# alexxx-db/dbx-distributed-pytorch-examples

Measured on AMD Instinct MI355X. Metric: images/sec (whole node) ResNet-50 ImageNet-1K at 1/2/4/8 MI355X; top-1 acc, higher is better.
Workload: dtype bf16; 1 GPU; model=resnet50 ImageNet-1K 224x224 1000 classes large-batch (global 8192 at 8 GPUs), global_batch=1024, per_gpu_batch=1024, parallelism=dp1, world_size_seen=1, backend=none, impl=native, optimizer=SGD momentum 0.9 nesterov=False wd 5e-5, memory_format=nhwc, graphs=True, ddp=none, kernels=dbx HIP (conv implicit-GEMM MFMA + fused BN/ReLU/pool/CE/SGD)

## Files before the change

### dbx_distributed_pytorch_examples_amd/csrc/abi.h

```cpp
#pragma once
typedef __bf16 bf16;
namespace dbx {
struct BnFin {
  unsigned* cnt;
  const double* stats;
  const float* gamma;
  const float* beta;
  float* running_mean;
  float* running_var;
  float* scale;
  float* shift;
  float* mean;
  float* invstd;
  float* coeff;
  float* dgamma;
  float* dbeta;
  int C, nshard, mode, accumulate;
  float count, eps, momentum, pad_;
};
struct IGemmArgs {
  const bf16* x;
  const bf16* w;
  bf16* y;
  const float* in_scale;
// ... 9 lines not shown
  const bf16* ybn;
  const bf16* ybn2;
  const float* bsc;
  const float* bsh;
  const float* mean1;
  const float* inv1;
  const float* mean2;
  const float* inv2;
  double* bstats1;
  double* bstats2;
  bf16* a_out;
  const bf16* res;
  const float* res_scale;
  const float* res_shift;
  bf16* tail_out;
  unsigned char* tail_bits;
  unsigned long long mag_ohw, mag_ow;
  const BnFin* fin1;
  const BnFin* fin2;
  int fin_base, fin_final;
  const BnFin* fin_in;
  float* skws;
  unsigned* skcnt;
  int ksplit, kper;
};
struct WgradArgs {
  const bf16* dy;
  const bf16* x;
  float* ws;
  const float* in_scale;
  const float* in_shift;
  int N, IH, IW, IC, OH, OW, OC, R, S, stride, pad;
  int M, KTOT, nsplit, m_per_split, relu_in;
  unsigned long long mag_ow, mag_ohw;
  float* dw;
  unsigned* cnt;
  float scale;
  int accumulate;
};
struct DwFusedArgs {
  const bf16* g;
  const bf16* y3;
  const float* coeff;
  const bf16* wt;
  const bf16* y2;
  const float* bsc;
  const float* bsh;
  const float* mean2;
  const float* inv2;
  bf16* da;
  double* bstats;
  float* ws;
  int M, K, C, nshard;
};
struct StemBwdArgs {
  const bf16* dpool;
  const unsigned char* arg;
  const bf16* y;
  const float* sc;
  const float* sh;
  const float* coeff;
  const bf16* x4;
  float* ws;
  int N, H, W, C, P, Q, PK, pstride, ppad;
  int IH, IW, R, S, stride, pad;
  int M, nsplit, m_per_split;
  unsigned long long mag_hw, mag_w;
};
struct GemmArgs {
  const bf16* A;
  const bf16* B;
  void* C;
  const float* bias_f;
  const bf16* bias_h;
  int M, N, K, lda, ldb, ldc;
  float alpha;
  int accumulate;
  unsigned long long seed;
  unsigned offset, thresh;
  float inv_keep;
  const unsigned* offset_dev;
  float* ws;
  int splitk;
};

}
```

### dbx_distributed_pytorch_examples_amd/csrc/bindings.cpp

```cpp
#include <hip/hip_runtime.h>
#include <pybind11/pybind11.h>
#include <pybind11/stl.h>
#include <stdint.h>

#include <stdexcept>
#include <string>

namespace py = pybind11;
#include "abi.h"

extern "C" {
int dbx_conv_igemm(int mode, int bm, int bn, const dbx::IGemmArgs* a, int pro, int stats, int accum, int epi,
                   hipStream_t st, int dma);
int dbx_conv_wgrad(int mode, int bm, int bn, const dbx::WgradArgs* a, int pro, hipStream_t st, unsigned lds_pad,
                   int dma);
int dbx_wgrad_reduce_multi_plan(const float* const*, float* const*, const long long*, const int*, const float*,
                                const int*, int, void*, int*, int*);
int dbx_wgrad_reduce_multi_run(const void*, int, int, int, hipStream_t);
int dbx_wgrad_reduce_job_bytes();
int dbx_wgrad_reduce(const float* ws, float* dw, long long n, int nsplit, float scale, int accumulate, hipStream_t st);
int dbx_wgrad_reduce_gather(const float* ws, float* dw, int OC, int R, int S, int IC, int nsplit, float scale,
                            int accumulate, hipStream_t st);
int dbx_wgrad_patch3(const dbx::WgradArgs* a, long long ws_cap, hipStream_t st, int max_wg);
int dbx_conv_dwfused(const dbx::DwFusedArgs* a, long long ws_cap, hipStream_t st, int max_cus);
// ... 105 lines not shown
    if (fin2 && !bstats2) throw std::invalid_argument("conv_igemm: second BN finalize without its statistics");
    {
      const unsigned long long two40 = 1ull << 40, ohw = (unsigned long long)OH * OW;
      if (ohw > 0 && (unsigned long long)N * ohw * ohw < two40) {
        a.mag_ohw = (two40 + ohw - 1) / ohw;
        a.mag_ow = (two40 + OW - 1) / OW;
      }
    }
    check(dbx_conv_igemm(mode, bm, bn, &a, in_scale != 0, stats != 0, accum, epi, S(st), dma), "conv_igemm");
  });
  m.def("wgrad_reduce_multi_plan", [](std::vector<uintptr_t> ws, std::vector<uintptr_t> dw, std::vector<long long> n,
                                       std::vector<int> nsplit, std::vector<float> scale, std::vector<int> acc,
                                       uintptr_t table) {
    const size_t nj = ws.size();
    if (dw.size() != nj || n.size() != nj || nsplit.size() != nj || scale.size() != nj || acc.size() != nj)
      throw std::invalid_argument("wgrad_reduce_multi_plan: job lists of different lengths");
    std::vector<const float*> w(nj);
    std::vector<float*> d(nj);
    for (size_t q = 0; q < nj; ++q) { w[q] = P<const float*>(ws[q]); d[q] = P<float*>(dw[q]); }
    int ga = 0, gb = 0;
    check(dbx_wgrad_reduce_multi_plan(w.data(), d.data(), n.data(), nsplit.data(), scale.data(), acc.data(), (int)nj,
                                      P<void*>(table), &ga, &gb),
          "wgrad_reduce_multi_plan");
    return std::make_pair(ga, gb);
  });
  m.def("wgrad_reduce_multi_run", [](uintptr_t table_dev, int nj, int ga, int gb, uintptr_t st) {
    check(dbx_wgrad_reduce_multi_run(P<const void*>(table_dev), nj, ga, gb, S(st)), "wgrad_reduce_multi_run");
  });
  m.def("wgrad_reduce_job_bytes", []() { return dbx_wgrad_reduce_job_bytes(); });
  m.def("conv_wgrad", [](int mode, int bm, int bn, uintptr_t dy, uintptr_t x, uintptr_t ws, uintptr_t in_scale,
                         uintptr_t in_shift, int relu_in, int N, int IH, int IW, int IC, int OH, int OW, int OC, int R,
                         int S_, int stride, int pad, int KTOT, int nsplit, int m_per_split, uintptr_t st,
                         unsigned lds_pad, int dma, uintptr_t dw, uintptr_t cnt, float scale, int accumulate) {
    const unsigned long long two40 = 1ull << 40;
    const unsigned long long ohw = (unsigned long long)OH * OW;
    if ((unsigned long long)N * ohw * ohw >= two40) throw std::runtime_error("conv_wgrad: batch too large for mdiv");
    dbx::WgradArgs a{P<const bf16*>(dy), P<const bf16*>(x), P<float*>(ws), P<const float*>(in_scale),
                     P<const float*>(in_shift), N, IH, IW, IC, OH, OW, OC, R, S_, stride, pad, N * OH * OW, KTOT,
                     nsplit, m_per_split, relu_in, (two40 + OW - 1) / OW, (two40 + ohw - 1) / ohw,
                     P<float*>(dw), P<unsigned*>(cnt), scale, accumulate};
    if (dw && nsplit > 1 && !cnt) throw std::invalid_argument("conv_wgrad: fused split-K reduction needs tile counters");
    check(dbx_conv_wgrad(mode, bm, bn, &a, in_scale != 0, S(st), lds_pad, dma), "conv_wgrad");
  });
  m.def("wgrad_patch3", [](uintptr_t dy, uintptr_t x, uintptr_t ws, long long ws_cap, int N, int IH, int IW, int IC,
                           int OH, int OW, int OC, int R, int S_, int stride, int pad, uintptr_t st, int max_wg) {
    dbx::WgradArgs a{P<const bf16*>(dy), P<const bf16*>(x), P<float*>(ws), nullptr, nullptr, N, IH, IW, IC, OH, OW,
                     OC, R, S_, stride, pad, N * OH * OW, R * S_ * IC, 0, 0, 0, 0ull, 0ull};
    const int n = dbx_wgrad_patch3(&a, ws_cap, S(st), max_wg);
    if (n <= 0) check(n ? n : -1, "wgrad_patch3");
    return n;
  });
  m.def("conv_dwfused", [](uintptr_t g, uintptr_t y3, uintptr_t coeff, uintptr_t wt, uintptr_t y2, uintptr_t bsc,
                           uintptr_t bsh, uintptr_t mean2, uintptr_t inv2, uintptr_t da, uintptr_t bstats, uintptr_t ws,
                           long long ws_cap, int M, int K, int C, int nshard, uintptr_t st, int max_cus) {
    dbx::DwFusedArgs a{P<const bf16*>(g), P<const bf16*>(y3), P<const float*>(coeff), P<const bf16*>(wt),
                       P<const bf16*>(y2), P<const float*>(bsc), P<const float*>(bsh), P<const float*>(mean2),
                       P<const float*>(inv2), P<bf16*>(da), P<double*>(bstats), P<float*>(ws), M, K, C,
                       nshard > 0 ? nshard : 1};
    const int n = dbx_conv_dwfused(&a, ws_cap, S(st), max_cus);
    if (n <= 0) check(n ? n : -1, "conv_dwfused");
    return n;
  });
  m.def("stem_bwd", [](uintptr_t dpool, uintptr_t arg, uintptr_t y, uintptr_t sc, uintptr_t sh, uintptr_t coeff,
                       uintptr_t x4, uintptr_t ws, long long ws_cap, int N, int H, int W, int C, int Pp, int Qq, int PK,
                       int pstride, int ppad, int IH, int IW, int R, int S_, int stride, int pad, int fused,
                       uintptr_t st) {
    const unsigned long long two40 = 1ull << 40, hw = (unsigned long long)H * W;
    if ((unsigned long long)N * hw * hw >= two40) throw std::runtime_error("stem_bwd: batch too large for mdiv");
    dbx::StemBwdArgs a{P<const bf16*>(dpool), P<const unsigned char*>(arg), P<const bf16*>(y), P<const float*>(sc),
                       P<const float*>(sh), P<const float*>(coeff), P<const bf16*>(x4), P<float*>(ws), N, H, W, C, Pp, Qq,
                       PK, pstride, ppad, IH, IW, R, S_, stride, pad, N * H * W, 0, 0, (two40 + hw - 1) / hw,
                       (two40 + W - 1) / W};
    const int n = dbx_stem_bwd(&a, ws_cap, fused, S(st));
    if (n <= 0) check(n ? n : -1, "stem_bwd");
    return n;
  });
  m.def("wgrad_reduce_gather", [](uintptr_t ws, uintptr_t dw, int OC, int R, int S_, int IC, int nsplit, float scale,
                                  int acc, uintptr_t st) {
    check(dbx_wgrad_reduce_gather(P<const float*>(ws), P<float*>(dw), OC, R, S_, IC, nsplit, scale, acc, S(st)),
          "wgrad_reduce_gather");
  });
  m.def("wgrad_reduce", [](uintptr_t ws, uintptr_t dw, long long n, int nsplit, float scale, int acc, uintptr_t st) {
    check(dbx_wgrad_reduce(P<const float*>(ws), P<float*>(dw), n, nsplit, scale, acc, S(st)), "wgrad_reduce");
  });
  m.def("bn_finalize", [](uintptr_t stats, int nshard, int C, float count, uintptr_t gamma, uintptr_t beta, float eps,
                          float momentum, uintptr_t rm, uintptr_t rv, uintptr_t scale, uintptr_t shift, uintptr_t smean,
                          uintptr_t sinv, uintptr_t st) {
    check(dbx_bn_finalize(P<const double*>(stats), nshard, C, count, P<const float*>(gamma), P<const float*>(beta), eps,
                          momentum, P<float*>(rm), P<float*>(rv), P<float*>(scale), P<float*>(shift), P<float*>(smean),
                          P<float*>(sinv), S(st)),
          "bn_finalize");
  });
  m.def("bn_eval_coeff", [](int C, uintptr_t gamma, uintptr_t beta, float eps, uintptr_t rm, uintptr_t rv,
                            uintptr_t scale, uintptr_t shift, uintptr_t st) {
    check(dbx_bn_eval_coeff(C, P<const float*>(gamma), P<const float*>(beta), eps, P<const float*>(rm),
                            P<const float*>(rv), P<float*>(scale), P<float*>(shift), S(st)),
          "bn_eval_coeff");
  });
  m.def("bn_eval_coeff_multi", [](uintptr_t desc, int nbn, int max_c, uintptr_t st) {
    check(dbx_bn_eval_coeff_multi(P<const void*>(desc), nbn, max_c, S(st)), "bn_eval_coeff_multi");
  });
  m.def("ce_eval", [](uintptr_t logits, int is_bf16, uintptr_t labels, uintptr_t stats, int B, int C, int k,
                      uintptr_t nvalid, uintptr_t loss_out, uintptr_t rank_out, uintptr_t st) {
    check(dbx_ce_eval(P<const void*>(logits), is_bf16, P<const long long*>(labels), P<double*>(stats), B, C, k,
                      P<const int*>(nvalid), P<float*>(loss_out), P<int*>(rank_out), S(st)),
          "ce_eval");
  });
  m.def("channel_stats", [](uintptr_t y, long long M, int C, uintptr_t stats, int nshard, uintptr_t st) {
    check(dbx_channel_stats(P<const bf16*>(y), M, C, P<double*>(stats), nshard, S(st)), "channel_stats");
  });
  m.def("bn_apply", [](uintptr_t y, uintptr_t sc, uintptr_t sh, uintptr_t res, uintptr_t rsc, uintptr_t rsh,
// ... 201 lines not shown
```

### dbx_distributed_pytorch_examples_amd/csrc/conv_dwfused.hip

```cpp
#include "common.h"
#include "abi.h"

namespace dbx {

template <int C, int NKB, int BM, int NS, int NT, int WN, int OCC, bool Y2N>
__global__ __launch_bounds__(NT, OCC) void dwfused_kernel(const DwFusedArgs a) {
  constexpr int K = NKB * 64;
  constexpr int NW = NT / 64, WM = NW / WN;
  constexpr int WC = C / WN;
  constexpr int WCH = K / 8;
  constexpr int CPR = C / 8;
  constexpr int RPP = NT / CPR;
  constexpr int NY = BM / RPP;
  constexpr int LR = NT / 8;
  constexpr int NG = BM / LR;
  constexpr int TM = BM / (16 * WM), TN = WC / 16;
  constexpr int TNW = WC / 16;
  static_assert(NKB % NS == 0 && C % 64 == 0 && WM == 2 && BM % (16 * WM) == 0 && BM % LR == 0 && BM % RPP == 0,
                "tile shape");
  constexpr int LDS_W = C * K, LDS_A = 2 * BM * 64, LDS_P = BM * C;
  static_assert(BM * (C + 8) <= LDS_A + LDS_P, "epilogue staging must fit the dy3 + a2 images");
  __shared__ __attribute__((aligned(16))) bf16 lds[LDS_W + LDS_A + LDS_P];
  bf16* sW = lds;
  bf16* sA = lds + LDS_W;
  bf16* sP = sA + LDS_A;
  bf16* sC = sA;

  const int tid = threadIdx.x, lane = tid & 63, wid = tid >> 6, wm = wid / WN, wn = wid % WN;
  const int ntile = a.M / BM;
  const int lrow = tid >> 3, lch = tid & 7;
  const int erow = tid / CPR, ech = tid % CPR;

  for (int q = tid; q < C * WCH; q += NT) {
    const int row = q / WCH, ch = q - (q / WCH) * WCH;
    *reinterpret_cast<u32x4*>(sW + row * K + ((ch ^ (row & 15)) << 3)) =
        *reinterpret_cast<const u32x4*>(a.wt + (size_t)row * K + ch * 8);
  }
  int cbn = ech * 8;
  auto bn2_affine = [&](f32x4& s0, f32x4& s1, f32x4& h0, f32x4& h1) __attribute__((always_inline)) {
    asm volatile("" : "+v"(cbn));
    s0 = *reinterpret_cast<const f32x4*>(a.bsc + cbn);
    s1 = *reinterpret_cast<const f32x4*>(a.bsc + cbn + 4);
    h0 = *reinterpret_cast<const f32x4*>(a.bsh + cbn);
    h1 = *reinterpret_cast<const f32x4*>(a.bsh + cbn + 4);
  };
  f32x2 st_s[4], st_q[4];
#pragma unroll
  for (int h = 0; h < 4; ++h) st_s[h] = st_q[h] = f32x2{0.f, 0.f};
  f32x4 accw[NKB][2][TNW];
#pragma unroll
  for (int kb = 0; kb < NKB; ++kb)
#pragma unroll
    for (int i = 0; i < 2; ++i)
#pragma unroll
      for (int j = 0; j < TNW; ++j) accw[kb][i][j] = f32x4{0.f, 0.f, 0.f, 0.f};

  const rsrc_t gr = make_rsrc(a.g, 2ull * a.M * K);
  const rsrc_t yr = make_rsrc(a.y3, 2ull * a.M * K);
  const rsrc_t y2r = make_rsrc(a.y2, 2ull * a.M * C);
  u32x4 rg[NS][NG], ry[NS][NG], ry2[NY], ry2n[Y2N ? NY : 1];
  auto load_k = [&](int t, int kb, int set) __attribute__((always_inline)) {
#pragma unroll
    for (int i = 0; i < NG; ++i) {
      const unsigned off = t < ntile ? 2u * (unsigned)((t * BM + lrow + LR * i) * K + kb * 64 + lch * 8) : kOOB;
      rg[set][i] = buf_load16(gr, off);
      ry[set][i] = buf_load16(yr, off);
    }
  };
  auto y2_off = [&](int t, int i) __attribute__((always_inline)) {
    return t < ntile ? 2u * (unsigned)((t * BM + erow + RPP * i) * C + ech * 8) : kOOB;
  };
  auto fold_store = [&](int kb, int buf, int set) __attribute__((always_inline)) {
    const int c0 = kb * 64 + lch * 8;
    const f32x4 k1a = *reinterpret_cast<const f32x4*>(a.coeff + c0);
    const f32x4 k1b = *reinterpret_cast<const f32x4*>(a.coeff + c0 + 4);
    const f32x4 k2a = *reinterpret_cast<const f32x4*>(a.coeff + K + c0);
    const f32x4 k2b = *reinterpret_cast<const f32x4*>(a.coeff + K + c0 + 4);
    const f32x4 k3a = *reinterpret_cast<const f32x4*>(a.coeff + 2 * K + c0);
    const f32x4 k3b = *reinterpret_cast<const f32x4*>(a.coeff + 2 * K + c0 + 4);
#pragma unroll
    for (int i = 0; i < NG; ++i) {
      float f[8], y[8];
      unpack8(rg[set][i], f);
      unpack8(ry[set][i], y);
#pragma unroll
      for (int j = 0; j < 4; ++j) {
        f[j] = f[j] * k1a[j] + k3a[j] + y[j] * k2a[j];
        f[j + 4] = f[j + 4] * k1b[j] + k3b[j] + y[j + 4] * k2b[j];
      }
      const int row = lrow + LR * i;
      *reinterpret_cast<u32x4*>(sA + buf * BM * 64 + row * 64 + (tr_swz(row, lch, 8) << 3)) = pack8(f);
    }
  };
  auto a2_store = [&]() __attribute__((always_inline)) {
    f32x4 bsc0, bsc1, bsh0, bsh1;
    bn2_affine(bsc0, bsc1, bsh0, bsh1);
#pragma unroll
    for (int i = 0; i < NY; ++i) {
      float f[8];
      unpack8(ry2[i], f);
#pragma unroll
      for (int j = 0; j < 4; ++j) {
        f[j] = f[j] * bsc0[j] + bsh0[j];
        f[j + 4] = f[j + 4] * bsc1[j] + bsh1[j];
      }
      const int row = erow + RPP * i;
      *reinterpret_cast<u32x4*>(sP + row * C + (tr_swz(row, ech, CPR) << 3)) = relu_bf16x8(pack8(f));
    }
  };

  const int g4 = lane >> 4, q4 = (lane & 15) >> 2, p4 = lane & 3;
  f32x4 accd[TM][TN];
  auto mma = [&](int kb, int buf) __attribute__((always_inline)) {
    const bf16* cA = sA + buf * BM * 64;
#pragma unroll
    for (int ks = 0; ks < 2; ++ks) {
      const int ch = ks * 4 + g4;
      bf16x8 af[TM], bw[TN];
#pragma unroll
      for (int i = 0; i < TM; ++i) {
        const int row = wm * (BM / WM) + i * 16 + (lane & 15);
        af[i] = *reinterpret_cast<const bf16x8*>(cA + row * 64 + (tr_swz(row, ch, 8) << 3));
      }
#pragma unroll
      for (int j = 0; j < TN; ++j) {
        const int crow = wn * WC + j * 16 + (lane & 15);
        bw[j] = *reinterpret_cast<const bf16x8*>(sW + crow * K + (((kb * 8 + ch) ^ (crow & 15)) << 3));
      }
#pragma unroll
      for (int i = 0; i < TM; ++i)
#pragma unroll
        for (int j = 0; j < TN; ++j)
          accd[i][j] = __builtin_amdgcn_mfma_f32_16x16x32_bf16(bw[j], af[i], accd[i][j], 0, 0, 0);
    }
#pragma unroll
    for (int ks = 0; ks < BM / 32; ++ks) {
      const int row = ks * 32 + 8 * g4 + q4, row2 = row + 4;
      bf16x8 af[2], bp[TNW];
#pragma unroll
      for (int i = 0; i < 2; ++i) {
        const int col = wm * 32 + i * 16 + 4 * p4;
        const s16x4 lo = __builtin_amdgcn_ds_read_tr16_b64_v4i16(
            (DBX_LDS s16x4*)(cA + row * 64 + (tr_swz(row, col >> 3, 8) << 3) + (col & 7)));
        const s16x4 hi = __builtin_amdgcn_ds_read_tr16_b64_v4i16(
            (DBX_LDS s16x4*)(cA + row2 * 64 + (tr_swz(row2, col >> 3, 8) << 3) + (col & 7)));
        af[i] = __builtin_bit_cast(bf16x8, __builtin_shufflevector(lo, hi, 0, 1, 2, 3, 4, 5, 6, 7));
      }
#pragma unroll
      for (int j = 0; j < TNW; ++j) {
        const int col = wn * WC + j * 16 + 4 * p4;
        const s16x4 lo = __builtin_amdgcn_ds_read_tr16_b64_v4i16(
            (DBX_LDS s16x4*)(sP + row * C + (tr_swz(row, col >> 3, CPR) << 3) + (col & 7)));
        const s16x4 hi = __builtin_amdgcn_ds_read_tr16_b64_v4i16(
            (DBX_LDS s16x4*)(sP + row2 * C + (tr_swz(row2, col >> 3, CPR) << 3) + (col & 7)));
        bp[j] = __builtin_bit_cast(bf16x8, __builtin_shufflevector(lo, hi, 0, 1, 2, 3, 4, 5, 6, 7));
      }
#pragma unroll
      for (int i = 0; i < 2; ++i)
#pragma unroll
        for (int j = 0; j < TNW; ++j)
          accw[kb][i][j] = __builtin_amdgcn_mfma_f32_16x16x32_bf16(af[i], bp[j], accw[kb][i][j], 0, 0, 0);
    }
  };

  int t = blockIdx.x;
#pragma unroll
  for (int i = 0; i < NY; ++i) ry2[i] = buf_load16(y2r, y2_off(t, i));
#pragma unroll
  for (int s = 0; s < NS; ++s) load_k(t, s, s);
  __syncthreads();
  for (; t < ntile; t += gridDim.x) {
    const int tn = t + gridDim.x;
    if constexpr (Y2N) {
#pragma unroll
      for (int i = 0; i < NY; ++i) ry2n[i] = buf_load16(y2r, y2_off(tn, i));
    }
    a2_store();
    fold_store(0, 0, 0);
    __syncthreads();
#pragma unroll
    for (int i = 0; i < TM; ++i)
#pragma unroll
      for (int j = 0; j < TN; ++j) accd[i][j] = f32x4{0.f, 0.f, 0.f, 0.f};
#pragma unroll
    for (int kb = 0; kb < NKB; ++kb) {
      const int f = kb + NS;
      load_k(f < NKB ? t : tn, f < NKB ? f : f - NKB, kb % NS);
      mma(kb, kb & 1);
      if (kb + 1 < NKB) fold_store(kb + 1, (kb + 1) & 1, (kb + 1) % NS);
      __syncthreads();
    }
#pragma unroll
    for (int i = 0; i < TM; ++i)
#pragma unroll
      for (int j = 0; j < TN; ++j) {
        const int row = wm * (BM / WM) + i * 16 + (lane & 15);
        const int col = wn * WC + j * 16 + g4 * 4;
        *reinterpret_cast<uint2*>(sC + row * (C + 8) + col) =
            uint2{pack2(accd[i][j][0], accd[i][j][1]), pack2(accd[i][j][2], accd[i][j][3])};
      }
    __syncthreads();
    f32x4 bsc0, bsc1, bsh0, bsh1;
    bn2_affine(bsc0, bsc1, bsh0, bsh1);
#pragma unroll
    for (int i = 0; i < NY; ++i) {
      const int row = erow + RPP * i;
      float f[8], y[8];
      unpack8(*reinterpret_cast<const u32x4*>(sC + row * (C + 8) + ech * 8), f);
      unpack8(ry2[i], y);
#pragma unroll
      for (int j = 0; j < 4; ++j) {
        const float t0 = y[j] * bsc0[j] + bsh0[j], t1 = y[j + 4] * bsc1[j] + bsh1[j];
        f[j] = t0 > 0.f ? f[j] : 0.f;
        f[j + 4] = t1 > 0.f ? f[j + 4] : 0.f;
      }
      const u32x4 v = pack8(f);
      *reinterpret_cast<u32x4*>(a.da + (size_t)(t * BM + row) * C + ech * 8) = v;
#pragma unroll
      for (int h = 0; h < 4; ++h) {
        const f32x2 gv = {__uint_as_float(v[h] << 16), __uint_as_float(v[h] & 0xFFFF0000u)};
        const f32x2 yv = {__uint_as_float(ry2[i][h] << 16), __uint_as_float(ry2[i][h] & 0xFFFF0000u)};
        st_s[h] += gv;
        st_q[h] = __builtin_elementwise_fma(gv, yv, st_q[h]);
      }
      if constexpr (Y2N) ry2[i] = ry2n[i];
      else ry2[i] = buf_load16(y2r, y2_off(tn, i));
    }
    __syncthreads();
  }

  float* out = a.ws + (size_t)blockIdx.x * K * C;
#pragma unroll
  for (int kb = 0; kb < NKB; ++kb)
#pragma unroll
    for (int i = 0; i < 2; ++i)
#pragma unroll
      for (int j = 0; j < TNW; ++j)
#pragma unroll
        for (int r = 0; r < 4; ++r) {
          const int k = kb * 64 + wm * 32 + i * 16 + g4 * 4 + r;
          out[(size_t)k * C + wn * WC + j * 16 + (lane & 15)] = accw[kb][i][j][r];
        }
  float s[8], q[8];
#pragma unroll
  for (int h = 0; h < 4; ++h) {
    s[2 * h] = st_s[h].x; s[2 * h + 1] = st_s[h].y;
    q[2 * h] = st_q[h].x; q[2 * h + 1] = st_q[h].y;
  }
#pragma unroll
  for (int j = 0; j < 8; ++j)
#pragma unroll
    for (int o = CPR; o < 64; o <<= 1) {
      s[j] += __shfl_xor(s[j], o, 64);
      q[j] += __shfl_xor(q[j], o, 64);
    }
  float* red = reinterpret_cast<float*>(sA);
  if (lane < CPR) {
#pragma unroll
    for (int j = 0; j < 8; ++j) {
      red[(wid * 2 + 0) * C + lane * 8 + j] = s[j];
      red[(wid * 2 + 1) * C + lane * 8 + j] = q[j];
    }
  }
  __syncthreads();
  for (int c = tid; c < C; c += NT) {
    float ss = 0.f, qq = 0.f;
#pragma unroll
    for (int w = 0; w < NW; ++w) { ss += red[(w * 2) * C + c]; qq += red[(w * 2 + 1) * C + c]; }
    qq = a.inv2[c] * (qq - a.mean2[c] * ss);
    double* st = a.bstats + (size_t)(blockIdx.x % a.nshard) * 2 * C;
    atomicAdd(st + c, (double)ss);
    atomicAdd(st + C + c, (double)qq);
  }
}

}

using namespace dbx;

template <int C, int NKB, int BM, int NS, int NT, int WN, int OCC, bool Y2N>
static int launch_dwfused(const DwFusedArgs& a, long long ws_cap, hipStream_t st, int max_cus) {
  if (a.M % BM != 0 || a.M <= 0) return -31;
  struct Occ { int per_cu, cus; };
  static const Occ occ = [] {
    int per_cu = 0, dev = 0, cus = 0;
    (void)hipOccupancyMaxActiveBlocksPerMultiprocessor(
        &per_cu, reinterpret_cast<const void*>(&dwfused_kernel<C, NKB, BM, NS, NT, WN, OCC, Y2N>), NT, 0);
    (void)hipGetDevice(&dev);
    (void)hipDeviceGetAttribute(&cus, hipDeviceAttributeMultiprocessorCount, dev);
    return Occ{per_cu, cus};
  }();
  const int cus = (max_cus > 0 && max_cus < occ.cus) ? (max_cus & ~7) : occ.cus;
  const int cap = (occ.per_cu > 0 && cus > 0) ? occ.per_cu * cus : 256;
  const int ntile = a.M / BM;
  const int grid = ntile < cap ? ntile : cap;
  if ((long long)(grid + (grid < 64 ? grid : 64)) * a.K * a.C > ws_cap) return -33;
  hipLaunchKernelGGL((dwfused_kernel<C, NKB, BM, NS, NT, WN, OCC, Y2N>), dim3(grid), dim3(NT), 0, st, a);
  const hipError_t e = hipGetLastError();
  return e == hipSuccess ? grid : -(int)e - 1000;
}

extern "C" int dbx_conv_dwfused(const DwFusedArgs* args, long long ws_cap, hipStream_t st, int max_cus) {
  const DwFusedArgs& a = *args;
  if (2ull * a.M * a.K >= (unsigned long long)kOOB) return -32;
#ifndef DBX_DWF64
#define DBX_DWF64 64, 2, 256, 2, 2, false
#endif
  if (a.C == 64 && a.K == 256) return launch_dwfused<64, 4, DBX_DWF64>(a, ws_cap, st, max_cus);
#ifndef DBX_DWF128
#define DBX_DWF128 64, 2, 256, 2, 1, false
#endif
  if (a.C == 128 && a.K == 512) return launch_dwfused<128, 8, DBX_DWF128>(a, ws_cap, st, max_cus);
  return -30;
}
```

### dbx_distributed_pytorch_examples_amd/ops/kernels.py

```python
from __future__ import annotations

import os
from typing import Optional, Tuple

import torch

from ..utils import debug as _debug
from . import reference as _ref
from ._ext import C, stream_ptr, use_native
from ..engine_config import EngineConfig

_E = EngineConfig.current

FWD, DGRAD, STEM, FWD_PATCH, DGRAD_PATCH = 0, 1, 2, 3, 4
_NO_EPI = (0, 1, 0, 0, 0, 0, 0, 0, 0, 0, 0, 0, 0, 0)
MASK_NONE, MASK_OUT, MASK_Y = 0, 1, 2


_POST_LAUNCH = None


def set_post_launch(cb, owner=None) -> None:
    global _POST_LAUNCH
    if cb is None and owner is not None and _POST_LAUNCH is not None and _POST_LAUNCH != owner:
# ... 683 lines not shown
                              cus=num_cus() - cu_reserve if cu_reserve > 0 else None)
    if (nsplit + (min(64, nsplit) if nsplit > 8 else 0)) * OC * KTOT > ws.numel():
        raise ValueError("wgrad workspace too small")
    fuse = not stem and (nsplit == 1 or (cnt is not None and nsplit * bm * bn * 4 <= wgrad_fuse_max()))
    if fuse and nsplit > 1:
        _chk(cnt, torch.int32, "cnt")
        if cnt.numel() < (OC // bm) * (KTOT // bn):
            raise ValueError("conv_wgrad: tile counter slice too small")
    region = None
    if (defer is not None and not fuse and (defer.max_slab_bytes is None
                                           or 4 * nsplit * OC * KTOT <= defer.max_slab_bytes)):
        region = defer.alloc((nsplit + (min(64, nsplit) if nsplit > 8 else 0)) * OC * KTOT)
        if region is not None:
            ws = region
    C().conv_wgrad(STEM if stem else FWD, bm, bn, dy.data_ptr(), x.data_ptr(), ws.data_ptr(), _p(in_scale),
                   _p(in_shift), int(relu_in), N, IH, IW, IC, OH, OW, OC, R, S, stride, pad, KTOT, nsplit, ms,
                   stream_ptr(), int(lds_pad), int(dma), dw.data_ptr() if fuse else 0,
                   cnt.data_ptr() if fuse and cnt is not None else 0, float(scale), int(accumulate))
    if region is not None:
        defer.add(ws, dw, OC * KTOT, nsplit, scale, accumulate)
    elif not fuse:
        C().wgrad_reduce(ws.data_ptr(), dw.data_ptr(), OC * KTOT, nsplit, float(scale), int(accumulate), stream_ptr())
    return dw


def dwfused_supported(C: int, K: int, M: int) -> bool:
    return (C, K) in ((64, 256), (128, 512)) and M % 64 == 0 and 2 * M * K < 0xFFFFFF00


def num_cus() -> int:
    global _NUM_CUS
    if _NUM_CUS is None:
        try:
            _NUM_CUS = int(torch.cuda.get_device_properties(torch.cuda.current_device()).multi_processor_count) \
                if torch.cuda.is_available() else 256
        except Exception:
            _NUM_CUS = 256
    return _NUM_CUS


_NUM_CUS = None


def dwfused_grid(C: int, K: int) -> int:
    return (2 if (C, K) == (64, 256) else 1) * num_cus()


def dwfused_preferred(C: int, K: int, M: int) -> bool:
    grid = dwfused_grid(C, K)
    return dwfused_supported(C, K, M) and M >= _E().fuse_dw_min_tiles * grid * 64


@_dispatch
def conv_dwfused(g, y3, coeff, wt16, y2, scale2, shift2, mean2, invstd2, bstats2, da, dw, ws, cus: int = 0):
    N, H, W, Kc = g.shape
    Cc = y2.shape[-1]
    M = N * H * W
    _chk(g, torch.bfloat16, "g")
    _chk(y3, torch.bfloat16, "y3", g.numel())
    _chk(coeff, torch.float32, "coeff", 3 * Kc)
    _chk(wt16, torch.bfloat16, "wt16", Cc * Kc)
    _chk(y2, torch.bfloat16, "y2", M * Cc)
    _chk(da, torch.bfloat16, "da", M * Cc)
    _chk(dw, torch.float32, "dw", Kc * Cc)
    _chk(ws, torch.float32, "ws")
    nsh2 = _chk_stats(bstats2, "bstats2", Cc)
    for t, nm in ((scale2, "scale2"), (shift2, "shift2"), (mean2, "mean2"), (invstd2, "invstd2")):
        _chk(t, torch.float32, nm, Cc)
    if not dwfused_supported(Cc, Kc, M):
        raise ValueError(f"conv_dwfused: unsupported geometry C={Cc} K={Kc} M={M}")
    n = C().conv_dwfused(g.data_ptr(), y3.data_ptr(), coeff.data_ptr(), wt16.data_ptr(), y2.data_ptr(),
                         scale2.data_ptr(), shift2.data_ptr(), mean2.data_ptr(), invstd2.data_ptr(), da.data_ptr(),
                         bstats2.data_ptr(), ws.data_ptr(), ws.numel(), M, Kc, Cc, nsh2, stream_ptr(), int(cus))
    C().wgrad_reduce(ws.data_ptr(), dw.data_ptr(), Kc * Cc, n, 1.0, 0, stream_ptr())
    return da


@_dispatch
def bn_finalize(stats, count, gamma, beta, eps, momentum, running_mean, running_var, scale, shift,
                save_mean, save_invstd):
    Cc = scale.numel()
    C().bn_finalize(stats.data_ptr(), _nsh(stats, Cc), Cc, float(count), _p(gamma), _p(beta), float(eps), float(momentum),
                    _p(running_mean), _p(running_var), scale.data_ptr(), shift.data_ptr(), _p(save_mean),
                    _p(save_invstd), stream_ptr())


@_dispatch
def bn_eval_coeff(gamma, beta, eps, running_mean, running_var, scale, shift):
    C().bn_eval_coeff(scale.numel(), _p(gamma), _p(beta), float(eps), running_mean.data_ptr(),
                      running_var.data_ptr(), scale.data_ptr(), shift.data_ptr(), stream_ptr())


def pack_bn_eval_desc(entries, device) -> torch.Tensor:
    import numpy as np
    want = torch.device(device)
    rows = np.zeros(len(entries), dtype=_ref.bn_eval_desc_dtype())
    for i, (gamma, beta, eps, rm, rv, scale, shift) in enumerate(entries):
        n = scale.numel()
        for t, nm in ((gamma, "gamma"), (beta, "beta"), (rm, "running_mean"), (rv, "running_var"), (scale, "scale"),
                      (shift, "shift")):
            if t is None and nm in ("gamma", "beta"):
                continue
            if t.dtype != torch.float32:
                raise TypeError(f"pack_bn_eval_desc: entry {i} {nm}: expected torch.float32, got {t.dtype}")
            same_dev = t.device.type == want.type and (want.index is None or t.device.index == want.index)
            if not t.is_contiguous() or not same_dev:
                raise ValueError(f"pack_bn_eval_desc: entry {i} {nm}: must be contiguous and on {device}")
            if t.numel() != n:
                raise ValueError(f"pack_bn_eval_desc: entry {i} {nm}: {t.numel()} elements, scale has {n}")
        rows[i] = ([_p(gamma), _p(beta), rm.data_ptr(), rv.data_ptr(), scale.data_ptr(), shift.data_ptr()], n, eps)
    table = torch.from_numpy(rows.view(np.uint8).copy()).to(device)
    return table, len(entries), max((int(r["C"]) for r in rows), default=0)


@_dispatch
def bn_eval_coeff_multi(desc, nbn, max_c):
    if desc.dtype != torch.uint8:
        raise TypeError(f"desc: expected torch.uint8, got {desc.dtype}")
    if not desc.is_contiguous() or desc.numel() != _ref.BN_EVAL_DESC_BYTES * int(nbn):
        raise ValueError(f"desc: expected a contiguous [{nbn}, {_ref.BN_EVAL_DESC_BYTES}] byte table, got shape "
                         f"{tuple(desc.shape)}")
    C().bn_eval_coeff_multi(desc.data_ptr(), int(nbn), int(max_c), stream_ptr())


@_dispatch
def channel_stats(y, stats):
# ... 539 lines not shown
```

### dbx_distributed_pytorch_examples_amd/ops/reference.py

```python
from __future__ import annotations

import math

import torch
import torch.nn.functional as F

NSHARD = 32
MASK_NONE, MASK_OUT, MASK_Y = 0, 1, 2


def check_channels(C: int) -> None:
    if C < 8 or C % 8 or C // 8 > 256:
        raise ValueError(f"per-channel kernels need a channel count that is a multiple of 8, at most 2048; got {C}")


def _shards(stats, C: int):
    n = stats.numel() // (2 * C)
    if n < 1 or n > 32 or n * 2 * C != stats.numel():
        raise ValueError(f"statistics slab of {stats.numel()} elements is not [nshard <= 32, 2, {C}]")
    return stats.view(n, 2, C)


def _nchw(x):
    return x.permute(0, 3, 1, 2)
# ... 73 lines not shown
        else:
            t = y * e.scale + e.shift
            g = g * (t > 0)
            if getattr(e, "act_out", None) is not None:
                e.act_out.copy_(torch.relu(t).bfloat16())
        g = g.bfloat16().float()
        gf = g.reshape(-1, Cc)
        st = e.stats1.view(-1, 2, Cc)
        st[0, 0] += gf.sum(0)
        st[0, 1] += (gf * ((y - e.mean1) * e.inv1).reshape(-1, Cc)).sum(0)
        if e.ybn2 is not None:
            st2 = e.stats2.view(-1, 2, Cc)
            st2[0, 0] += gf.sum(0)
            st2[0, 1] += (gf * ((e.ybn2.float() - e.mean2) * e.inv2).reshape(-1, Cc)).sum(0)
        if hasattr(e, "run_fin"):
            e.run_fin()
    dx.copy_(g.bfloat16())
    return dx


def conv_stem_fwd(x4, w16s, out, *, R=7, S=7, stride=2, pad=3, stats=None, patch=None):
    OC = w16s.shape[0]
    w = w16s.float().view(OC, 8, 8, 4)[:, :R, :S, :].permute(0, 3, 1, 2)
    y = _nhwc(F.conv2d(_nchw(x4.float()), w, stride=stride, padding=pad)).bfloat16()
    out.copy_(y)
    if stats is not None:
        _add_stats(stats, out)
    return out


def conv_wgrad(dy, x, dw, ws, *, R, S, stride, pad, in_scale=None, in_shift=None, relu_in=True, scale=1.0,
               accumulate=False, stem=False, tile=None, lds_pad=0, dma=-1, cnt=None, out_krsc=None, rounds=None,
               defer=None, cu_reserve=0):
    N, OH, OW, OC = dy.shape
    IC = x.shape[-1]
    xf = _act_in(x, in_scale, in_shift, relu_in)
    g = torch.nn.grad.conv2d_weight(_nchw(xf), (OC, IC, R, S), _nchw(dy.float()), stride=stride, padding=pad)
    g = g.permute(0, 2, 3, 1) * scale
    if stem and out_krsc is not None:
        icr = out_krsc.numel() // (OC * R * S)
        out_krsc.copy_((g[..., :icr].reshape(-1) + (out_krsc if accumulate else 0)))
        return out_krsc
    if stem:
        full = torch.zeros(OC, 8, 8, 4, dtype=torch.float32, device=dy.device)
        full[:, :R, :S, :IC] = g
        g = full
    g = g.reshape(dw.shape)
    if accumulate:
        g = g + dw
    dw.copy_(g)
    return dw


def conv_dwfused(g, y3, coeff, wt16, y2, scale2, shift2, mean2, invstd2, bstats2, da, dw, ws, cus=0):
    from types import SimpleNamespace
    dy = torch.empty_like(g)
    bn_bwd_apply(g, y3, coeff, dy, mask_mode=MASK_NONE)
    act = torch.relu(y2.float() * scale2 + shift2).bfloat16()
    epi = SimpleNamespace(mode=MASK_Y, ybn=y2, mean1=mean2, inv1=invstd2, stats1=bstats2, mbits=None, scale=scale2,
                          shift=shift2, ybn2=None, mean2=None, inv2=None, stats2=None, act_out=None)
    conv_dgrad(dy, wt16, da, R=1, S=1, stride=1, pad=0, epilogue=epi)
    conv_wgrad(dy, act, dw, ws, R=1, S=1, stride=1, pad=0)
    return da


def bn_finalize(stats, count, gamma, beta, eps, momentum, running_mean, running_var, scale, shift, save_mean,
                save_invstd):
    C = scale.numel()
    st = _shards(stats, C).double().sum(0)
    mean = st[0] / count
    var = (st[1] / count - mean * mean).clamp_min(0)
    invstd = 1.0 / torch.sqrt(var + eps)
    g = gamma.double() if gamma is not None else torch.ones_like(mean)
    b = beta.double() if beta is not None else torch.zeros_like(mean)
    scale.copy_((g * invstd).float())
    shift.copy_((b - mean * g * invstd).float())
    if save_mean is not None:
        save_mean.copy_(mean.float())
    if save_invstd is not None:
        save_invstd.copy_(invstd.float())
    if running_mean is not None and momentum > 0:
        unb = var * count / (count - 1) if count > 1 else var
        running_mean.mul_(1 - momentum).add_(momentum * mean.float())
        running_var.mul_(1 - momentum).add_(momentum * unb.float())


def bn_eval_coeff(gamma, beta, eps, running_mean, running_var, scale, shift):
    inv = torch.rsqrt(running_var + eps)
    g = gamma if gamma is not None else torch.ones_like(inv)
    b = beta if beta is not None else torch.zeros_like(inv)
    scale.copy_(g * inv)
    shift.copy_(b - running_mean * g * inv)


BN_EVAL_DESC_BYTES = 56


def bn_eval_desc_dtype():
    import numpy as np
    return np.dtype([("ptr", np.int64, (6,)), ("C", np.int32), ("eps", np.float32)])


def bn_eval_coeff_multi(desc, nbn, max_c):
    import ctypes
    if desc.dtype != torch.uint8 or desc.numel() != BN_EVAL_DESC_BYTES * int(nbn):
        raise ValueError("bn_eval_coeff_multi: expected a uint8 [nbn, 56] table")

# ... 569 lines not shown
```

Measured before the change: 17050 images/s.

## Split C=128 dwfused kernel into two channel-half slices with persistent slab walk

For the C=128, K=512 fused dgrad/wgrad backward kernel, the default path now launches a C=64-sliced variant in which paired blocks each handle one channel half of the same M tiles, walking slabs persistently. BN coefficients and scale/shift are staged in LDS, and the transposed activation fragments are loaded once per tile. The goal is to cut per-block LDS and register footprint and raise parallelism. The cost is that g/y3 loads and the fold work are repeated across the two halves. The old kernel remains reachable with variant=1.

Result: no change. 17130 images/s, median of 6 (+0.5%).

```diff
diff --git a/dbx_distributed_pytorch_examples_amd/csrc/abi.h b/dbx_distributed_pytorch_examples_amd/csrc/abi.h
--- a/dbx_distributed_pytorch_examples_amd/csrc/abi.h
+++ b/dbx_distributed_pytorch_examples_amd/csrc/abi.h
@@ -85,6 +85,8 @@
   double* bstats;
   float* ws;
   int M, K, C, nshard;
+  int variant;
+  int nwalk;
 };
 struct StemBwdArgs {
   const bf16* dpool;
diff --git a/dbx_distributed_pytorch_examples_amd/csrc/bindings.cpp b/dbx_distributed_pytorch_examples_amd/csrc/bindings.cpp
--- a/dbx_distributed_pytorch_examples_amd/csrc/bindings.cpp
+++ b/dbx_distributed_pytorch_examples_amd/csrc/bindings.cpp
@@ -181,11 +181,11 @@
   });
   m.def("conv_dwfused", [](uintptr_t g, uintptr_t y3, uintptr_t coeff, uintptr_t wt, uintptr_t y2, uintptr_t bsc,
                            uintptr_t bsh, uintptr_t mean2, uintptr_t inv2, uintptr_t da, uintptr_t bstats, uintptr_t ws,
-                           long long ws_cap, int M, int K, int C, int nshard, uintptr_t st, int max_cus) {
+                           long long ws_cap, int M, int K, int C, int nshard, uintptr_t st, int max_cus, int variant) {
     dbx::DwFusedArgs a{P<const bf16*>(g), P<const bf16*>(y3), P<const float*>(coeff), P<const bf16*>(wt),
                        P<const bf16*>(y2), P<const float*>(bsc), P<const float*>(bsh), P<const float*>(mean2),
                        P<const float*>(inv2), P<bf16*>(da), P<double*>(bstats), P<float*>(ws), M, K, C,
-                       nshard > 0 ? nshard : 1};
+                       nshard > 0 ? nshard : 1, variant};
     const int n = dbx_conv_dwfused(&a, ws_cap, S(st), max_cus);
     if (n <= 0) check(n ? n : -1, "conv_dwfused");
     return n;
diff --git a/dbx_distributed_pytorch_examples_amd/csrc/conv_dwfused.hip b/dbx_distributed_pytorch_examples_amd/csrc/conv_dwfused.hip
--- a/dbx_distributed_pytorch_examples_amd/csrc/conv_dwfused.hip
+++ b/dbx_distributed_pytorch_examples_amd/csrc/conv_dwfused.hip
@@ -3,14 +3,17 @@
 
 namespace dbx {
 
-template <int C, int NKB, int BM, int NS, int NT, int WN, int OCC, bool Y2N>
+template <int C, int NKB, int BM, int NS, int NT, int WN, int OCC, bool Y2N, int CT = C>
 __global__ __launch_bounds__(NT, OCC) void dwfused_kernel(const DwFusedArgs a) {
   constexpr int K = NKB * 64;
+  static_assert(CT == C || CT == 2 * C, "slicing");
+  constexpr bool SL = CT != C;
   constexpr int NW = NT / 64, WM = NW / WN;
   constexpr int WC = C / WN;
   constexpr int WCH = K / 8;
   constexpr int CPR = C / 8;
-  constexpr int RPP = NT / CPR;
+  constexpr int ET = SL ? 128 : NT;
+  constexpr int RPP = ET / CPR;
   constexpr int NY = BM / RPP;
   constexpr int LR = NT / 8;
   constexpr int NG = BM / LR;
@@ -20,44 +23,53 @@
                 "tile shape");
   constexpr int LDS_W = C * K, LDS_A = 2 * BM * 64, LDS_P = BM * C;
   static_assert(BM * (C + 8) <= LDS_A + LDS_P, "epilogue staging must fit the dy3 + a2 images");
-  __shared__ __attribute__((aligned(16))) bf16 lds[LDS_W + LDS_A + LDS_P];
+  constexpr int LDS_X = SL ? 2 * (3 * K + 2 * C) : 0;
+  __shared__ __attribute__((aligned(16))) bf16 lds[LDS_W + LDS_A + LDS_P + LDS_X];
   bf16* sW = lds;
   bf16* sA = lds + LDS_W;
   bf16* sP = sA + LDS_A;
   bf16* sC = sA;
+  float* sX = reinterpret_cast<float*>(sP + LDS_P);
 
   const int tid = threadIdx.x, lane = tid & 63, wid = tid >> 6, wm = wid / WN, wn = wid % WN;
   const int ntile = a.M / BM;
   const int lrow = tid >> 3, lch = tid & 7;
   const int erow = tid / CPR, ech = tid % CPR;
+  const bool ep = !SL || tid < ET;
+  const int half = SL ? (blockIdx.x >> 3) & 1 : 0;
+  int slab = SL ? ((blockIdx.x >> 4) << 3) + (blockIdx.x & 7) : blockIdx.x;
+  const int tstep = SL ? a.nwalk : gridDim.x;
+  const int coff = half * C;
+  if (SL && slab >= a.nwalk) return;
 
   for (int q = tid; q < C * WCH; q += NT) {
     const int row = q / WCH, ch = q - (q / WCH) * WCH;
     *reinterpret_cast<u32x4*>(sW + row * K + ((ch ^ (row & 15)) << 3)) =
-        *reinterpret_cast<const u32x4*>(a.wt + (size_t)row * K + ch * 8);
-  }
-  int cbn = ech * 8;
+        *reinterpret_cast<const u32x4*>(a.wt + (size_t)(coff + row) * K + ch * 8);
+  }
+  if constexpr (SL) {
+    for (int q = tid; q < 3 * K; q += NT) sX[q] = a.coeff[q];
+    for (int q = tid; q < C; q += NT) {
+      sX[3 * K + q] = a.bsc[coff + q];
+      sX[3 * K + C + q] = a.bsh[coff + q];
+    }
+  }
+  int cbn = SL ? 3 * K + ech * 8 : ech * 8;
+  const float* pbsc = SL ? sX : a.bsc;
+  const float* pbsh = SL ? sX + C : a.bsh;
   auto bn2_affine = [&](f32x4& s0, f32x4& s1, f32x4& h0, f32x4& h1) __attribute__((always_inline)) {
     asm volatile("" : "+v"(cbn));
-    s0 = *reinterpret_cast<const f32x4*>(a.bsc + cbn);
-    s1 = *reinterpret_cast<const f32x4*>(a.bsc + cbn + 4);
-    h0 = *reinterpret_cast<const f32x4*>(a.bsh + cbn);
-    h1 = *reinterpret_cast<const f32x4*>(a.bsh + cbn + 4);
+    s0 = *reinterpret_cast<const f32x4*>(pbsc + cbn);
+    s1 = *reinterpret_cast<const f32x4*>(pbsc + cbn + 4);
+    h0 = *reinterpret_cast<const f32x4*>(pbsh + cbn);
+    h1 = *reinterpret_cast<const f32x4*>(pbsh + cbn + 4);
   };
   f32x2 st_s[4], st_q[4];
-#pragma unroll
-  for (int h = 0; h < 4; ++h) st_s[h] = st_q[h] = f32x2{0.f, 0.f};
   f32x4 accw[NKB][2][TNW];
-#pragma unroll
-  for (int kb = 0; kb < NKB; ++kb)
-#pragma unroll
-    for (int i = 0; i < 2; ++i)
-#pragma unroll
-      for (int j = 0; j < TNW; ++j) accw[kb][i][j] = f32x4{0.f, 0.f, 0.f, 0.f};
 
   const rsrc_t gr = make_rsrc(a.g, 2ull * a.M * K);
   const rsrc_t yr = make_rsrc(a.y3, 2ull * a.M * K);
-  const rsrc_t y2r = make_rsrc(a.y2, 2ull * a.M * C);
+  const rsrc_t y2r = make_rsrc(a.y2, 2ull * a.M * CT);
   u32x4 rg[NS][NG], ry[NS][NG], ry2[NY], ry2n[Y2N ? NY : 1];
   auto load_k = [&](int t, int kb, int set) __attribute__((always_inline)) {
 #pragma unroll
@@ -68,16 +80,18 @@
     }
   };
   auto y2_off = [&](int t, int i) __attribute__((always_inline)) {
-    return t < ntile ? 2u * (unsigned)((t * BM + erow + RPP * i) * C + ech * 8) : kOOB;
+    return (t < ntile && ep) ? 2u * (unsigned)((t * BM + erow + RPP * i) * CT + coff + ech * 8) : kOOB;
   };
   auto fold_store = [&](int kb, int buf, int set) __attribute__((always_inline)) {
-    const int c0 = kb * 64 + lch * 8;
-    const f32x4 k1a = *reinterpret_cast<const f32x4*>(a.coeff + c0);
-    const f32x4 k1b = *reinterpret_cast<const f32x4*>(a.coeff + c0 + 4);
-    const f32x4 k2a = *reinterpret_cast<const f32x4*>(a.coeff + K + c0);
-    const f32x4 k2b = *reinterpret_cast<const f32x4*>(a.coeff + K + c0 + 4);
-    const f32x4 k3a = *reinterpret_cast<const f32x4*>(a.coeff + 2 * K + c0);
-    const f32x4 k3b = *reinterpret_cast<const f32x4*>(a.coeff + 2 * K + c0 + 4);
+    int c0 = kb * 64 + lch * 8;
+    if constexpr (SL) asm volatile("" : "+v"(c0));
+    const float* pk = SL ? sX : a.coeff;
+    const f32x4 k1a = *reinterpret_cast<const f32x4*>(pk + c0);
+    const f32x4 k1b = *reinterpret_cast<const f32x4*>(pk + c0 + 4);
+    const f32x4 k2a = *reinterpret_cast<const f32x4*>(pk + K + c0);
+    const f32x4 k2b = *reinterpret_cast<const f32x4*>(pk + K + c0 + 4);
+    const f32x4 k3a = *reinterpret_cast<const f32x4*>(pk + 2 * K + c0);
+    const f32x4 k3b = *reinterpret_cast<const f32x4*>(pk + 2 * K + c0 + 4);
 #pragma unroll
     for (int i = 0; i < NG; ++i) {
       float f[8], y[8];
@@ -111,6 +125,22 @@
 
   const int g4 = lane >> 4, q4 = (lane & 15) >> 2, p4 = lane & 3;
   f32x4 accd[TM][TN];
+  int wsw[2][2];
+#pragma unroll
+  for (int p = 0; p < 2; ++p)
+#pragma unroll
+    for (int ks = 0; ks < 2; ++ks)
+      wsw[p][ks] = (wn * WC + (lane & 15)) * K + (((p * 8 + ks * 4 + g4) ^ (lane & 15)) << 3);
+  bf16x8 bpt[SL ? BM / 32 : 1][TNW];
+  auto load_bp = [&](int ks, int j) __attribute__((always_inline)) {
+    const int row = ks * 32 + 8 * g4 + q4, row2 = row + 4;
+    const int col = wn * WC + j * 16 + 4 * p4;
+    const s16x4 lo = __builtin_amdgcn_ds_read_tr16_b64_v4i16(
+        (DBX_LDS s16x4*)(sP + row * C + (tr_swz(row, col >> 3, CPR) << 3) + (col & 7)));
+    const s16x4 hi = __builtin_amdgcn_ds_read_tr16_b64_v4i16(
+        (DBX_LDS s16x4*)(sP + row2 * C + (tr_swz(row2, col >> 3, CPR) << 3) + (col & 7)));
+    return __builtin_bit_cast(bf16x8, __builtin_shufflevector(lo, hi, 0, 1, 2, 3, 4, 5, 6, 7));
+  };
   auto mma = [&](int kb, int buf) __attribute__((always_inline)) {
     const bf16* cA = sA + buf * BM * 64;
 #pragma unroll
@@ -125,7 +155,8 @@
 #pragma unroll
       for (int j = 0; j < TN; ++j) {
         const int crow = wn * WC + j * 16 + (lane & 15);
-        bw[j] = *reinterpret_cast<const bf16x8*>(sW + crow * K + (((kb * 8 + ch) ^ (crow & 15)) << 3));
+        if constexpr (SL) bw[j] = *reinterpret_cast<const bf16x8*>(sW + wsw[kb & 1][ks] + j * 16 * K + (kb >> 1) * 128);
+        else bw[j] = *reinterpret_cast<const bf16x8*>(sW + crow * K + (((kb * 8 + ch) ^ (crow & 15)) << 3));
       }
 #pragma unroll
       for (int i = 0; i < TM; ++i)
@@ -147,14 +178,7 @@
         af[i] = __builtin_bit_cast(bf16x8, __builtin_shufflevector(lo, hi, 0, 1, 2, 3, 4, 5, 6, 7));
       }
 #pragma unroll
-      for (int j = 0; j < TNW; ++j) {
-        const int col = wn * WC + j * 16 + 4 * p4;
-        const s16x4 lo = __builtin_amdgcn_ds_read_tr16_b64_v4i16(
-            (DBX_LDS s16x4*)(sP + row * C + (tr_swz(row, col >> 3, CPR) << 3) + (col & 7)));
-        const s16x4 hi = __builtin_amdgcn_ds_read_tr16_b64_v4i16(
-            (DBX_LDS s16x4*)(sP + row2 * C + (tr_swz(row2, col >> 3, CPR) << 3) + (col & 7)));
-        bp[j] = __builtin_bit_cast(bf16x8, __builtin_shufflevector(lo, hi, 0, 1, 2, 3, 4, 5, 6, 7));
-      }
+      for (int j = 0; j < TNW; ++j) bp[j] = SL ? bpt[SL ? ks : 0][j] : load_bp(ks, j);
 #pragma unroll
       for (int i = 0; i < 2; ++i)
 #pragma unroll
@@ -163,21 +187,36 @@
     }
   };
 
-  int t = blockIdx.x;
+  __syncthreads();
+  do {
+#pragma unroll
+  for (int h = 0; h < 4; ++h) st_s[h] = st_q[h] = f32x2{0.f, 0.f};
+#pragma unroll
+  for (int kb = 0; kb < NKB; ++kb)
+#pragma unroll
+    for (int i = 0; i < 2; ++i)
+#pragma unroll
+      for (int j = 0; j < TNW; ++j) accw[kb][i][j] = f32x4{0.f, 0.f, 0.f, 0.f};
+  int t = slab;
 #pragma unroll
   for (int i = 0; i < NY; ++i) ry2[i] = buf_load16(y2r, y2_off(t, i));
 #pragma unroll
   for (int s = 0; s < NS; ++s) load_k(t, s, s);
-  __syncthreads();
-  for (; t < ntile; t += gridDim.x) {
-    const int tn = t + gridDim.x;
+  for (; t < ntile; t += tstep) {
+    const int tn = t + tstep;
     if constexpr (Y2N) {
 #pragma unroll
       for (int i = 0; i < NY; ++i) ry2n[i] = buf_load16(y2r, y2_off(tn, i));
     }
-    a2_store();
+    if (ep) a2_store();
     fold_store(0, 0, 0);
     __syncthreads();
+    if constexpr (SL) {
+#pragma unroll
+      for (int ks = 0; ks < BM / 32; ++ks)
+#pragma unroll
+        for (int j = 0; j < TNW; ++j) bpt[ks][j] = load_bp(ks, j);
+    }
 #pragma unroll
     for (int i = 0; i < TM; ++i)
 #pragma unroll
@@ -204,6 +243,7 @@
     bn2_affine(bsc0, bsc1, bsh0, bsh1);
 #pragma unroll
     for (int i = 0; i < NY; ++i) {
+      if (!ep) break;
       const int row = erow + RPP * i;
       float f[8], y[8];
       unpack8(*reinterpret_cast<const u32x4*>(sC + row * (C + 8) + ech * 8), f);
@@ -215,7 +255,7 @@
         f[j + 4] = t1 > 0.f ? f[j + 4] : 0.f;
       }
       const u32x4 v = pack8(f);
-      *reinterpret_cast<u32x4*>(a.da + (size_t)(t * BM + row) * C + ech * 8) = v;
+      *reinterpret_cast<u32x4*>(a.da + (size_t)(t * BM + row) * CT + coff + ech * 8) = v;
 #pragma unroll
       for (int h = 0; h < 4; ++h) {
         const f32x2 gv = {__uint_as_float(v[h] << 16), __uint_as_float(v[h] & 0xFFFF0000u)};
@@ -229,7 +269,7 @@
     __syncthreads();
   }
 
-  float* out = a.ws + (size_t)blockIdx.x * K * C;
+  float* out = a.ws + (size_t)slab * K * CT + coff;
 #pragma unroll
   for (int kb = 0; kb < NKB; ++kb)
 #pragma unroll
@@ -239,7 +279,7 @@
 #pragma unroll
         for (int r = 0; r < 4; ++r) {
           const int k = kb * 64 + wm * 32 + i * 16 + g4 * 4 + r;
-          out[(size_t)k * C + wn * WC + j * 16 + (lane & 15)] = accw[kb][i][j][r];
+          out[(size_t)k * CT + wn * WC + j * 16 + (lane & 15)] = accw[kb][i][j][r];
         }
   float s[8], q[8];
 #pragma unroll
@@ -250,42 +290,47 @@
 #pragma unroll
   for (int j = 0; j < 8; ++j)
 #pragma unroll
-    for (int o = CPR; o < 64; o <<= 1) {
+    for (int o = CPR; o < (SL ? 32 : 64); o <<= 1) {
       s[j] += __shfl_xor(s[j], o, 64);
       q[j] += __shfl_xor(q[j], o, 64);
     }
+  constexpr int NR = SL ? 4 : NW;
   float* red = reinterpret_cast<float*>(sA);
-  if (lane < CPR) {
+  const int rch = SL ? lane & 31 : lane, ridx = SL ? wid * 2 + (lane >> 5) : wid;
+  if (ep && rch < CPR) {
 #pragma unroll
     for (int j = 0; j < 8; ++j) {
-      red[(wid * 2 + 0) * C + lane * 8 + j] = s[j];
-      red[(wid * 2 + 1) * C + lane * 8 + j] = q[j];
+      red[(ridx * 2 + 0) * C + rch * 8 + j] = s[j];
+      red[(ridx * 2 + 1) * C + rch * 8 + j] = q[j];
     }
   }
   __syncthreads();
   for (int c = tid; c < C; c += NT) {
+    if constexpr (SL) asm volatile("" : "+v"(c));
     float ss = 0.f, qq = 0.f;
 #pragma unroll
-    for (int w = 0; w < NW; ++w) { ss += red[(w * 2) * C + c]; qq += red[(w * 2 + 1) * C + c]; }
-    qq = a.inv2[c] * (qq - a.mean2[c] * ss);
-    double* st = a.bstats + (size_t)(blockIdx.x % a.nshard) * 2 * C;
+    for (int w = 0; w < NR; ++w) { ss += red[(w * 2) * C + c]; qq += red[(w * 2 + 1) * C + c]; }
+    qq = a.inv2[coff + c] * (qq - a.mean2[coff + c] * ss);
+    double* st = a.bstats + (size_t)(slab % a.nshard) * 2 * CT + coff;
     atomicAdd(st + c, (double)ss);
-    atomicAdd(st + C + c, (double)qq);
-  }
+    atomicAdd(st + CT + c, (double)qq);
+  }
+  if constexpr (SL) __syncthreads();
+  } while (SL && (slab += gridDim.x >> 1) < a.nwalk);
 }
 
 }
 
 using namespace dbx;
 
-template <int C, int NKB, int BM, int NS, int NT, int WN, int OCC, bool Y2N>
+template <int C, int NKB, int BM, int NS, int NT, int WN, int OCC, bool Y2N, int CT = C>
 static int launch_dwfused(const DwFusedArgs& a, long long ws_cap, hipStream_t st, int max_cus) {
   if (a.M % BM != 0 || a.M <= 0) return -31;
   struct Occ { int per_cu, cus; };
   static const Occ occ = [] {
     int per_cu = 0, dev = 0, cus = 0;
     (void)hipOccupancyMaxActiveBlocksPerMultiprocessor(
-        &per_cu, reinterpret_cast<const void*>(&dwfused_kernel<C, NKB, BM, NS, NT, WN, OCC, Y2N>), NT, 0);
+        &per_cu, reinterpret_cast<const void*>(&dwfused_kernel<C, NKB, BM, NS, NT, WN, OCC, Y2N, CT>), NT, 0);
     (void)hipGetDevice(&dev);
     (void)hipDeviceGetAttribute(&cus, hipDeviceAttributeMultiprocessorCount, dev);
     return Occ{per_cu, cus};
@@ -293,11 +338,17 @@
   const int cus = (max_cus > 0 && max_cus < occ.cus) ? (max_cus & ~7) : occ.cus;
   const int cap = (occ.per_cu > 0 && cus > 0) ? occ.per_cu * cus : 256;
   const int ntile = a.M / BM;
-  const int grid = ntile < cap ? ntile : cap;
-  if ((long long)(grid + (grid < 64 ? grid : 64)) * a.K * a.C > ws_cap) return -33;
-  hipLaunchKernelGGL((dwfused_kernel<C, NKB, BM, NS, NT, WN, OCC, Y2N>), dim3(grid), dim3(NT), 0, st, a);
+  int grid = ntile < cap ? ntile : cap, slabs = grid;
+  DwFusedArgs b = a;
+  if constexpr (CT != C) {
+    slabs = b.nwalk = ntile < cus ? ntile : cus;
+    const int res = cap / 2 >= 8 ? (cap / 2) & ~7 : 8, want = (slabs + 7) & ~7;
+    grid = 2 * (want < res ? want : res);
+  }
+  if ((long long)(slabs + (slabs < 64 ? slabs : 64)) * a.K * a.C > ws_cap) return -33;
+  hipLaunchKernelGGL((dwfused_kernel<C, NKB, BM, NS, NT, WN, OCC, Y2N, CT>), dim3(grid), dim3(NT), 0, st, b);
   const hipError_t e = hipGetLastError();
-  return e == hipSuccess ? grid : -(int)e - 1000;
+  return e == hipSuccess ? slabs : -(int)e - 1000;
 }
 
 extern "C" int dbx_conv_dwfused(const DwFusedArgs* args, long long ws_cap, hipStream_t st, int max_cus) {
@@ -307,9 +358,12 @@
 #define DBX_DWF64 64, 2, 256, 2, 2, false
 #endif
   if (a.C == 64 && a.K == 256) return launch_dwfused<64, 4, DBX_DWF64>(a, ws_cap, st, max_cus);
-#ifndef DBX_DWF128
-#define DBX_DWF128 64, 2, 256, 2, 1, false
+  if (a.C == 128 && a.K == 512) {
+    if (a.variant == 1) return launch_dwfused<128, 8, 64, 2, 256, 2, 1, false>(a, ws_cap, st, max_cus);
+#ifndef DBX_DWF128S
+#define DBX_DWF128S 64, 4, 512, 4, 2, false
 #endif
-  if (a.C == 128 && a.K == 512) return launch_dwfused<128, 8, DBX_DWF128>(a, ws_cap, st, max_cus);
+    return launch_dwfused<64, 8, DBX_DWF128S, 128>(a, ws_cap, st, max_cus);
+  }
   return -30;
 }
diff --git a/dbx_distributed_pytorch_examples_amd/ops/kernels.py b/dbx_distributed_pytorch_examples_amd/ops/kernels.py
--- a/dbx_distributed_pytorch_examples_amd/ops/kernels.py
+++ b/dbx_distributed_pytorch_examples_amd/ops/kernels.py
@@ -759,7 +759,8 @@
 
 
 @_dispatch
-def conv_dwfused(g, y3, coeff, wt16, y2, scale2, shift2, mean2, invstd2, bstats2, da, dw, ws, cus: int = 0):
+def conv_dwfused(g, y3, coeff, wt16, y2, scale2, shift2, mean2, invstd2, bstats2, da, dw, ws, cus: int = 0,
+                 variant: int = 0):
     N, H, W, Kc = g.shape
     Cc = y2.shape[-1]
     M = N * H * W
@@ -778,7 +779,8 @@
         raise ValueError(f"conv_dwfused: unsupported geometry C={Cc} K={Kc} M={M}")
     n = C().conv_dwfused(g.data_ptr(), y3.data_ptr(), coeff.data_ptr(), wt16.data_ptr(), y2.data_ptr(),
                          scale2.data_ptr(), shift2.data_ptr(), mean2.data_ptr(), invstd2.data_ptr(), da.data_ptr(),
-                         bstats2.data_ptr(), ws.data_ptr(), ws.numel(), M, Kc, Cc, nsh2, stream_ptr(), int(cus))
+                         bstats2.data_ptr(), ws.data_ptr(), ws.numel(), M, Kc, Cc, nsh2, stream_ptr(), int(cus),
+                         int(variant))
     C().wgrad_reduce(ws.data_ptr(), dw.data_ptr(), Kc * Cc, n, 1.0, 0, stream_ptr())
     return da
 
diff --git a/dbx_distributed_pytorch_examples_amd/ops/reference.py b/dbx_distributed_pytorch_examples_amd/ops/reference.py
--- a/dbx_distributed_pytorch_examples_amd/ops/reference.py
+++ b/dbx_distributed_pytorch_examples_amd/ops/reference.py
@@ -149,7 +149,7 @@
     return dw
 
 
-def conv_dwfused(g, y3, coeff, wt16, y2, scale2, shift2, mean2, invstd2, bstats2, da, dw, ws, cus=0):
+def conv_dwfused(g, y3, coeff, wt16, y2, scale2, shift2, mean2, invstd2, bstats2, da, dw, ws, cus=0, variant=0):
     from types import SimpleNamespace
     dy = torch.empty_like(g)
     bn_bwd_apply(g, y3, coeff, dy, mask_mode=MASK_NONE)
```
